# knagrecha/saturn

Measured on AMD Instinct MI355X. Metric: samples_per_s, higher is better.
Workload: dtype bf16; 1 GPU; model=gptj-6b, global_batch=16, seq_len=512, parallelism=dp1, optimizer=fused_sgd

## Files before the change

### saturn_amd/models/gptj.py

```python

from __future__ import annotations


import os
from dataclasses import dataclass

import torch
import torch.nn as nn

from saturn_amd.ops.functional import (
    fused_gelu,
    FusedLayerNorm,
    apply_rope,
    causal_attention,
    fused_add3,
    fused_cross_entropy,
    rope_tables,
    FusedDropout,
    FusedEmbedding,
    gptj_mlp,
    mlp_fused_supported,
)


@dataclass
class GPTJConfig:
    vocab_size: int = 50400
    n_ctx: int = 512
    n_embd: int = 4096
    n_head: int = 16
    n_layer: int = 28
    rotary_dim: int = 64
    embd_pdrop: float = 0.0
    resid_pdrop: float = 0.0


class GPTJAttention(nn.Module):
    def __init__(self, cfg: GPTJConfig):
        super().__init__()
        self.n_head = cfg.n_head
        self.head_dim = cfg.n_embd // cfg.n_head
        self.rotary_dim = cfg.rotary_dim
        E = cfg.n_embd
        self.q_proj = nn.Linear(E, E, bias=False)
        self.k_proj = nn.Linear(E, E, bias=False)
        self.v_proj = nn.Linear(E, E, bias=False)
        self.out_proj = nn.Linear(E, E, bias=False)
        self.n_ctx = cfg.n_ctx
        self._rope_f32 = rope_tables(cfg.n_ctx, cfg.rotary_dim)

    def _rope(self, device):
        if self._rope_f32[0].device != device:
            self._rope_f32 = tuple(t.to(device) for t in self._rope_f32)
        return self._rope_f32

    def forward(self, x):
        B, T, E = x.shape
        H, D = self.n_head, self.head_dim
        q = self.q_proj(x).view(B, T, H, D)
        k = self.k_proj(x).view(B, T, H, D)
        v = self.v_proj(x).view(B, T, H, D)
        cos, sin = self._rope(x.device)
        q = apply_rope(q, cos, sin)
        k = apply_rope(k, cos, sin)
        q = q.transpose(1, 2)
        k = k.transpose(1, 2)
        v = v.transpose(1, 2)
        o = causal_attention(q, k, v)
        o = o.transpose(1, 2).reshape(B, T, -1)
        return self.out_proj(o)


class GPTJMLP(nn.Module):
    def __init__(self, cfg: GPTJConfig):
        super().__init__()
        E = cfg.n_embd
        self.fc_in = nn.Linear(E, 4 * E)
        self.fc_out = nn.Linear(4 * E, E)

    @staticmethod
    def _plain_linear(m) -> bool:
        return type(m) is nn.Linear and not (
            m._forward_hooks
            or m._forward_pre_hooks
            or m._backward_hooks
            or m._backward_pre_hooks
        )

    def _use_fused(self, x) -> bool:
        if os.environ.get("SAMD_MLP_FUSED", "1") == "0":
            return False
        fi, fo = self.fc_in, self.fc_out
        return (
            x.is_cuda
            and self._plain_linear(fi)
            and self._plain_linear(fo)
            and mlp_fused_supported(x, fi.weight, fi.bias, fo.weight, fo.bias)
        )

    def forward(self, x):
        if self._use_fused(x):
            fi, fo = self.fc_in, self.fc_out
            return gptj_mlp(x, fi.weight, fi.bias, fo.weight, fo.bias)
        return self.fc_out(fused_gelu(self.fc_in(x)))


class GPTJBlock(nn.Module):

    def __init__(self, cfg: GPTJConfig):
        super().__init__()
        self.ln_1 = FusedLayerNorm(cfg.n_embd)
        self.attn = GPTJAttention(cfg)
        self.mlp = GPTJMLP(cfg)
        self.drop = FusedDropout(cfg.resid_pdrop)

    def forward(self, x):
        h = self.ln_1(x)
        return fused_add3(x, self.drop(self.attn(h)), self.drop(self.mlp(h)))


class GPTJForCausalLM(nn.Module):
    def __init__(self, cfg: GPTJConfig):
        super().__init__()
        self.cfg = cfg
        self.wte = FusedEmbedding(cfg.vocab_size, cfg.n_embd)
        self.drop = FusedDropout(cfg.embd_pdrop)
        self.h = nn.ModuleList(GPTJBlock(cfg) for _ in range(cfg.n_layer))
        self.ln_f = FusedLayerNorm(cfg.n_embd)
        self.lm_head = nn.Linear(cfg.n_embd, cfg.vocab_size, bias=True)
        self.apply(self._init)

    @staticmethod
    def _init(m):
        if isinstance(m, nn.Linear):
            nn.init.normal_(m.weight, std=0.02)
            if m.bias is not None:
                nn.init.zeros_(m.bias)
        elif isinstance(m, nn.Embedding):
            nn.init.normal_(m.weight, std=0.02)

    def forward(self, input_ids):
        x = self.drop(self.wte(input_ids))
        for block in self.h:
            x = block(x)
        x = self.ln_f(x)
        return self.lm_head(x)


def pretraining_loss(logits, labels):
    return fused_cross_entropy(logits, labels, shift=True)


class _EmbedStage(nn.Module):
    def __init__(self, wte):
        super().__init__()
        self.wte = wte

    def forward(self, input_ids):
        return self.wte(input_ids)


class _HeadStage(nn.Module):
    def __init__(self, ln_f, lm_head):
        super().__init__()
        self.ln_f = ln_f
        self.lm_head = lm_head

    def forward(self, x):
        return self.lm_head(self.ln_f(x))


def as_sequential(model: GPTJForCausalLM) -> nn.Sequential:
    return nn.Sequential(
        _EmbedStage(model.wte), *model.h, _HeadStage(model.ln_f, model.lm_head)
    )


def get_gptj_model(kwargs=None):
    kwargs = kwargs or {}
    cfg = GPTJConfig(
        n_layer=kwargs.get("n_layer", 28),
        n_embd=kwargs.get("n_embd", 4096),
        n_head=kwargs.get("n_head", 16),
        n_ctx=kwargs.get("n_ctx", 512),
        vocab_size=kwargs.get("vocab_size", 50400),
        rotary_dim=kwargs.get("rotary_dim", 64),
        embd_pdrop=kwargs.get("embd_pdrop", 0.0),
        resid_pdrop=kwargs.get("resid_pdrop", 0.0),
    )
    torch.manual_seed(kwargs.get("seed", 0))
    return GPTJForCausalLM(cfg)


class SyntheticTokens(torch.utils.data.Dataset):

    def __init__(self, n: int, seq_len: int, vocab: int, seed: int = 1):
        g = torch.Generator().manual_seed(seed)
        self.data = torch.randint(0, vocab, (n, seq_len), generator=g)

    def __len__(self):
        return len(self.data)

    def __getitem__(self, i):
        return self.data[i]


def _collate(batch):
    x = torch.stack(batch)
    return x, x.clone()


def make_token_dataloader(batch_size=8, seq_len=512, vocab=50400, n_batches=64):
    def get_dataloader():
        return torch.utils.data.DataLoader(
            SyntheticTokens(batch_size * n_batches, seq_len, vocab),
            batch_size=batch_size,
            shuffle=False,
            collate_fn=_collate,
        )

    return get_dataloader
```

### saturn_amd/ops/csrc/bindings.cpp

```cpp

#include <torch/extension.h>
#include <vector>

namespace samd {
void fused_sgd(std::vector<at::Tensor> params, std::vector<at::Tensor> grads,
               std::vector<at::Tensor> moms, std::vector<at::Tensor> masters,
               double lr, double momentum, double weight_decay);
void fused_adam(std::vector<at::Tensor> params, std::vector<at::Tensor> grads,
                std::vector<at::Tensor> ms, std::vector<at::Tensor> vs,
                std::vector<at::Tensor> masters, double lr, double beta1,
                double beta2, double eps, double weight_decay, double bc1,
                double bc2);
std::vector<at::Tensor> norm_fwd(at::Tensor x, at::Tensor w,
                                 c10::optional<at::Tensor> b, double eps,
                                 bool rms);
std::vector<at::Tensor> norm_bwd(at::Tensor dy, at::Tensor x, at::Tensor w,
                                 at::Tensor mean, at::Tensor rstd, bool rms,
                                 bool needs_db);
std::vector<at::Tensor> ce_fwd(at::Tensor logits, at::Tensor targets,
                               int64_t Tr, int64_t ignore_index);
at::Tensor ce_bwd(at::Tensor logits, at::Tensor targets, at::Tensor lse,
                  at::Tensor dloss, int64_t Tr, int64_t ignore_index);
void rope_apply(at::Tensor y, at::Tensor x, at::Tensor cos_t, at::Tensor sin_t,
                int64_t t_len, int64_t t_off, bool half_style, bool backward);
at::Tensor gelu_fwd(at::Tensor x);
at::Tensor gelu_bwd(at::Tensor dy, at::Tensor x);
std::vector<at::Tensor> attn_fwd(at::Tensor q, at::Tensor k, at::Tensor v,
                                 bool causal, int64_t kv_len);
std::vector<at::Tensor> attn_bwd(at::Tensor dout, at::Tensor q, at::Tensor k,
                                 at::Tensor v, at::Tensor o, at::Tensor lse,
                                 bool causal, int64_t kv_len);
std::string attn_dispatch(int64_t T, int64_t D);
at::Tensor add3(at::Tensor a, at::Tensor b, at::Tensor c);
at::Tensor swiglu_fwd(at::Tensor gate, at::Tensor up);
std::vector<at::Tensor> swiglu_bwd(at::Tensor dout, at::Tensor gate,
                                   at::Tensor up);
at::Tensor embed_fwd(at::Tensor weight, at::Tensor idx);
at::Tensor embed_bwd(at::Tensor dout, at::Tensor idx, long vocab);
at::Tensor dropout_fwd(at::Tensor x, double p, long seed);
at::Tensor dropout_bwd(at::Tensor dout, double p, long seed);
std::vector<at::Tensor> moe_route_fwd(at::Tensor logits, int64_t top_k,
                                      at::ScalarType out_dtype);
at::Tensor moe_route_bwd(at::Tensor logits, at::Tensor ids,
                         at::Tensor dweights);
std::vector<at::Tensor> moe_sort(at::Tensor ids, int64_t n_expert);
at::Tensor moe_permute_fwd(at::Tensor x, at::Tensor order, int64_t top_k);
at::Tensor moe_permute_bwd(at::Tensor dxs, at::Tensor pos);
at::Tensor moe_combine_fwd(at::Tensor y, at::Tensor weights, at::Tensor pos);
std::vector<at::Tensor> moe_combine_bwd(at::Tensor dout, at::Tensor y,
                                        at::Tensor weights, at::Tensor pos);
std::vector<at::Tensor> mlp_act_bwd(at::Tensor d_act, at::Tensor pre,
                                    bool want_dT, bool want_aT);
std::vector<at::Tensor> transpose_colsum(at::Tensor x, bool want_sum);
std::vector<at::Tensor> mlp_bwd(at::Tensor g, at::Tensor h, at::Tensor pre,
                                at::Tensor W_in, at::Tensor W_out,
                                bool use_tn_in, bool use_tn_out);
}

PYBIND11_MODULE(TORCH_EXTENSION_NAME, m) {
  m.doc() = "saturn_amd hand-written CDNA4 (gfx950) kernels";
  m.def("fused_sgd", &samd::fused_sgd, "fused multi-tensor SGD");
  m.def("fused_adam", &samd::fused_adam, "fused multi-tensor AdamW");
  m.def("norm_fwd", &samd::norm_fwd, "LayerNorm/RMSNorm forward");
  m.def("norm_bwd", &samd::norm_bwd, "LayerNorm/RMSNorm backward");
  m.def("ce_fwd", &samd::ce_fwd, "fused cross-entropy forward");
  m.def("ce_bwd", &samd::ce_bwd, "fused cross-entropy backward");
  m.def("rope_apply", &samd::rope_apply,
        "fused rotary embedding (out-of-place, offset table rows)");
  m.def("gelu_fwd", &samd::gelu_fwd, "fused tanh-approx GELU forward");
  m.def("gelu_bwd", &samd::gelu_bwd, "fused tanh-approx GELU backward");
  m.def("attn_fwd", &samd::attn_fwd, "fused flash attention forward",
        py::arg("q"), py::arg("k"), py::arg("v"), py::arg("causal"),
        py::arg("kv_len") = -1);
  m.def("attn_dispatch", &samd::attn_dispatch,
        "kernel instantiations attn_fwd/attn_bwd launch for (padded T, D)",
        py::arg("T"), py::arg("D"));
  m.def("attn_bwd", &samd::attn_bwd, "fused flash attention backward",
        py::arg("dout"), py::arg("q"), py::arg("k"), py::arg("v"),
        py::arg("o"), py::arg("lse"), py::arg("causal"),
        py::arg("kv_len") = -1);
  m.def("add3", &samd::add3, "fused 3-way residual add");
  m.def("swiglu_fwd", &samd::swiglu_fwd, "fused silu(gate)*up");
  m.def("swiglu_bwd", &samd::swiglu_bwd, "fused SwiGLU backward");
  m.def("embed_fwd", &samd::embed_fwd, "token embedding gather");
  m.def("embed_bwd", &samd::embed_bwd, "embedding scatter-add backward");
  m.def("dropout_fwd", &samd::dropout_fwd, "counter-based fused dropout");
  m.def("dropout_bwd", &samd::dropout_bwd, "dropout backward (mask recompute)");
  m.def("moe_route_fwd", &samd::moe_route_fwd,
        "MoE softmax + top-k + renormalise (ties to the lower expert)");
  m.def("moe_route_bwd", &samd::moe_route_bwd, "MoE routing backward");
  m.def("moe_sort", &samd::moe_sort,
        "stable counting sort of (token, slot) pairs by expert");
  m.def("moe_permute_fwd", &samd::moe_permute_fwd,
        "gather token rows into expert order");
  m.def("moe_permute_bwd", &samd::moe_permute_bwd,
        "sum each token's k permuted rows");
  m.def("moe_combine_fwd", &samd::moe_combine_fwd,
        "weighted sum of each token's k expert rows");
  m.def("moe_combine_bwd", &samd::moe_combine_bwd,
        "combine backward: dy and fp32 dweights");
  m.def("mlp_act_bwd", &samd::mlp_act_bwd,
        "GELU backward + transposed d_pre / gelu(pre) + fp32 bias grad",
        py::arg("d_act"), py::arg("pre"), py::arg("want_dT") = true,
        py::arg("want_aT") = true);
  m.def("transpose_colsum", &samd::transpose_colsum,
        "bf16 transpose with optional fp32 column sums");
  m.def("mlp_bwd", &samd::mlp_bwd,
        "GPT-J MLP backward with TN-layout weight gradients");
}
```

### saturn_amd/ops/csrc/mlp_bwd.hip

```cpp

#include <torch/extension.h>
#include <ATen/hip/HIPContext.h>

#include "common.h"
#include "gelu_math.h"

namespace samd {

namespace {

constexpr int MB_TILE = 64;
constexpr int MB_ROW_ITERS = 4;
constexpr int MB_BLOCK = 256;

typedef c10::BFloat16 bf16_t;

__device__ __forceinline__ int img_dword(int c, int rp) {
  return c * 32 + (((rp >> 2) ^ (c >> 3)) << 2) + (rp & 3);
}
__device__ __forceinline__ int img_slot(int c, int mv) {
  return c * 8 + (mv ^ (c >> 3));
}

__device__ __forceinline__ float sum8_bf16(const uint4 v) {
  float s = us2f((unsigned short)(v.x & 0xffffu));
  s += us2f((unsigned short)(v.x >> 16));
  s += us2f((unsigned short)(v.y & 0xffffu));
  s += us2f((unsigned short)(v.y >> 16));
  s += us2f((unsigned short)(v.z & 0xffffu));
  s += us2f((unsigned short)(v.z >> 16));
  s += us2f((unsigned short)(v.w & 0xffffu));
  s += us2f((unsigned short)(v.w >> 16));
  return s;
}

__device__ __forceinline__ void store_colsums(float acc0, float acc1,
                                              float4* lds_sum,
                                              float* __restrict__ partial,
                                              long col0, long ncols) {
  const int tid = threadIdx.x;
#pragma unroll
  for (int off = 1; off < 8; off <<= 1) {
    acc0 += __shfl_xor(acc0, off, 64);
    acc1 += __shfl_xor(acc1, off, 64);
  }
  float* s = reinterpret_cast<float*>(lds_sum);
  if ((tid & 7) == 0) {
    s[tid >> 3] = acc0;
    s[(tid >> 3) + 32] = acc1;
  }
  __syncthreads();
  if (tid < MB_TILE / 4 && col0 + tid * 4 < ncols) {
    *reinterpret_cast<float4*>(partial + (long)blockIdx.y * ncols + col0 +
                               tid * 4) = lds_sum[tid];
  }
}

template <bool TN_IN, bool TN_OUT>
__global__ void __launch_bounds__(MB_BLOCK)
mlp_act_bwd_kernel(const bf16_t* __restrict__ d_act,
                   const bf16_t* __restrict__ pre, bf16_t* __restrict__ d_pre,
                   bf16_t* __restrict__ d_preT, bf16_t* __restrict__ act,
                   float* __restrict__ partial, long M, long F) {
  __shared__ uint4 img_d[MB_TILE * 8];
  __shared__ uint4 img_a[TN_OUT ? MB_TILE * 8 : 1];
  __shared__ float4 lds_sum[MB_TILE / 4];

  const int tid = threadIdx.x;
  const int cv = tid & 7;
  const int rp = tid >> 3;
  const int mv = tid & 7;
  const int cr = tid >> 3;
  const long col0 = (long)blockIdx.x * MB_TILE;
  const long col = col0 + cv * 8;
  const bool col_ok = col < F;

  float acc0 = 0.f, acc1 = 0.f;

  for (int it = 0; it < MB_ROW_ITERS; ++it) {
    const long row0 = ((long)blockIdx.y * MB_ROW_ITERS + it) * MB_TILE;
    if (row0 >= M) break;
    const long row = row0 + 2 * rp;
    const bool ok = col_ok && row < M;

    const short8v zero8 = {0, 0, 0, 0, 0, 0, 0, 0};
    short8v xv[2], gv[2];
#pragma unroll
    for (int i = 0; i < 2; ++i) {
      if (ok) {
        const long o = (row + i) * F + col;
        xv[i] = *reinterpret_cast<const short8v*>(pre + o);
        gv[i] = *reinterpret_cast<const short8v*>(d_act + o);
      } else {
        xv[i] = zero8;
        gv[i] = zero8;
      }
    }
    short8v dv[2], av[2];
#pragma unroll
    for (int i = 0; i < 2; ++i) {
#pragma unroll
      for (int e = 0; e < 8; ++e) {
        bf16_t xe, de;
        xe.x = (unsigned short)xv[i][e];
        de.x = (unsigned short)gv[i][e];
        const float xf = toF<bf16_t>(xe);
        dv[i][e] = (short)fromF<bf16_t>(toF<bf16_t>(de) * dgelu_f(xf)).x;
        av[i][e] = (short)fromF<bf16_t>(gelu_f(xf)).x;
      }
    }
    if (ok) {
#pragma unroll
      for (int i = 0; i < 2; ++i) {
        const long o = (row + i) * F + col;
        *reinterpret_cast<short8v*>(d_pre + o) = dv[i];
        if (!TN_OUT) *reinterpret_cast<short8v*>(act + o) = av[i];
      }
    }
    unsigned* d32 = reinterpret_cast<unsigned*>(img_d);
    unsigned* a32 = reinterpret_cast<unsigned*>(img_a);
#pragma unroll
    for (int e = 0; e < 8; ++e) {
      const int w = img_dword(cv * 8 + e, rp);
      d32[w] = ok ? ((unsigned)(unsigned short)dv[0][e] |
                     ((unsigned)(unsigned short)dv[1][e] << 16))
                  : 0u;
      if (TN_OUT)
        a32[w] = ok ? ((unsigned)(unsigned short)av[0][e] |
                       ((unsigned)(unsigned short)av[1][e] << 16))
                    : 0u;
    }
    __syncthreads();

    const long mrow = row0 + mv * 8;
#pragma unroll
    for (int j = 0; j < 2; ++j) {
      const int c = cr + 32 * j;
      const uint4 d = img_d[img_slot(c, mv)];
      const float s = sum8_bf16(d);
      if (j == 0) acc0 += s; else acc1 += s;
      const bool st = (col0 + c < F) && (mrow < M);
      if (TN_IN && st)
        *reinterpret_cast<uint4*>(d_preT + (col0 + c) * M + mrow) = d;
      if (TN_OUT && st)
        *reinterpret_cast<uint4*>(act + (col0 + c) * M + mrow) =
            img_a[img_slot(c, mv)];
    }
    __syncthreads();
  }
  store_colsums(acc0, acc1, lds_sum, partial, col0, F);
}

template <bool SUM, bool STORE>
__global__ void __launch_bounds__(MB_BLOCK)
transpose_colsum_kernel(const bf16_t* __restrict__ x, bf16_t* __restrict__ xT,
                        float* __restrict__ partial, long M, long N) {
  __shared__ uint4 img[MB_TILE * 8];
  __shared__ float4 lds_sum[MB_TILE / 4];

  const int tid = threadIdx.x;
  const int cv = tid & 7;
  const int rp = tid >> 3;
  const int mv = tid & 7;
  const int cr = tid >> 3;
  const long col0 = (long)blockIdx.x * MB_TILE;
  const long col = col0 + cv * 8;
  const bool col_ok = col < N;

  float acc0 = 0.f, acc1 = 0.f;

  for (int it = 0; it < MB_ROW_ITERS; ++it) {
    const long row0 = ((long)blockIdx.y * MB_ROW_ITERS + it) * MB_TILE;
    if (row0 >= M) break;
    const long row = row0 + 2 * rp;
    const bool ok = col_ok && row < M;

    const short8v zero8 = {0, 0, 0, 0, 0, 0, 0, 0};
    short8v xv[2];
#pragma unroll
    for (int i = 0; i < 2; ++i) {
      xv[i] = zero8;
      if (ok) xv[i] = *reinterpret_cast<const short8v*>(x + (row + i) * N + col);
    }
    unsigned* i32 = reinterpret_cast<unsigned*>(img);
#pragma unroll
    for (int e = 0; e < 8; ++e) {
      i32[img_dword(cv * 8 + e, rp)] =
          (unsigned)(unsigned short)xv[0][e] |
          ((unsigned)(unsigned short)xv[1][e] << 16);
    }
    __syncthreads();

    const long mrow = row0 + mv * 8;
#pragma unroll
    for (int j = 0; j < 2; ++j) {
      const int c = cr + 32 * j;
      const uint4 v = img[img_slot(c, mv)];
      if (SUM) {
        const float s = sum8_bf16(v);
        if (j == 0) acc0 += s; else acc1 += s;
      }
      if (STORE && (col0 + c < N) && (mrow < M))
        *reinterpret_cast<uint4*>(xT + (col0 + c) * M + mrow) = v;
    }
    __syncthreads();
  }
  if (SUM) store_colsums(acc0, acc1, lds_sum, partial, col0, N);
}

void check_operand(const at::Tensor& t, const char* name) {
  TORCH_CHECK(t.is_cuda(), name, ": expected a GPU tensor");
  TORCH_CHECK(t.scalar_type() == at::kBFloat16, name, ": expected bf16");
  TORCH_CHECK(t.dim() == 2 && t.is_contiguous(), name,
              ": expected a contiguous 2-D tensor");
  TORCH_CHECK(t.size(0) > 0 && t.size(0) % 8 == 0 && t.size(1) > 0 &&
                  t.size(1) % 8 == 0,
              name, ": both sizes must be positive multiples of 8, got ",
              t.sizes());
  TORCH_CHECK(reinterpret_cast<uintptr_t>(t.data_ptr()) % 16 == 0, name,
              ": data must be 16-byte aligned");
}

dim3 tile_grid(long M, long N) {
  const long gx = (N + MB_TILE - 1) / MB_TILE;
  const long gy = (M + MB_TILE * MB_ROW_ITERS - 1) / (MB_TILE * MB_ROW_ITERS);
  TORCH_CHECK(gy <= 65535, "mlp_bwd: too many rows for one launch");
  return dim3((unsigned)gx, (unsigned)gy);
}

bf16_t* bptr(const at::Tensor& t) {
  return reinterpret_cast<bf16_t*>(t.data_ptr());
}

}

std::vector<at::Tensor> mlp_act_bwd(at::Tensor d_act, at::Tensor pre,
                                    bool want_dT, bool want_aT) {
  check_operand(d_act, "mlp_act_bwd d_act");
  check_operand(pre, "mlp_act_bwd pre");
  TORCH_CHECK(d_act.sizes() == pre.sizes(), "mlp_act_bwd: shape mismatch");
  const long M = pre.size(0), F = pre.size(1);
  auto d_pre = at::empty_like(pre);
  auto d_preT = want_dT ? at::empty({F, M}, pre.options())
                        : at::empty({0}, pre.options());
  auto act = want_aT ? at::empty({F, M}, pre.options()) : at::empty_like(pre);
  const dim3 grid = tile_grid(M, F);
  auto partial =
      at::empty({(long)grid.y, F}, pre.options().dtype(at::kFloat));
  auto stream = at::hip::getCurrentHIPStream();
#define SAMD_LAUNCH_ACT_BWD(TI, TO)                                        \
  hipLaunchKernelGGL((mlp_act_bwd_kernel<TI, TO>), grid, dim3(MB_BLOCK), 0, \
                     stream.stream(), bptr(d_act), bptr(pre), bptr(d_pre),  \
                     want_dT ? bptr(d_preT) : nullptr, bptr(act),           \
                     partial.data_ptr<float>(), M, F)
  if (want_dT && want_aT) SAMD_LAUNCH_ACT_BWD(true, true);
  else if (want_dT) SAMD_LAUNCH_ACT_BWD(true, false);
  else if (want_aT) SAMD_LAUNCH_ACT_BWD(false, true);
  else SAMD_LAUNCH_ACT_BWD(false, false);
#undef SAMD_LAUNCH_ACT_BWD
  SAMD_CHECK_HIP(hipGetLastError());
  return {d_pre, d_preT, act, at::sum(partial, {0})};
}

namespace {

std::vector<at::Tensor> transpose_colsum_impl(const at::Tensor& x,
                                              bool want_sum, bool want_store) {
  check_operand(x, "transpose_colsum x");
  TORCH_CHECK(want_sum || want_store, "transpose_colsum: nothing to do");
  const long M = x.size(0), N = x.size(1);
  auto xT = want_store ? at::empty({N, M}, x.options())
                       : at::empty({0}, x.options());
  const dim3 grid = tile_grid(M, N);
  const auto fopt = x.options().dtype(at::kFloat);
  auto partial = want_sum ? at::empty({(long)grid.y, N}, fopt)
                          : at::empty({0}, fopt);
  auto stream = at::hip::getCurrentHIPStream();
#define SAMD_LAUNCH_TRANSPOSE(SUM, STORE)                                    \
  hipLaunchKernelGGL((transpose_colsum_kernel<SUM, STORE>), grid,            \
                     dim3(MB_BLOCK), 0, stream.stream(), bptr(x),            \
                     want_store ? bptr(xT) : nullptr,                        \
                     want_sum ? partial.data_ptr<float>() : nullptr, M, N)
  if (want_sum && want_store) SAMD_LAUNCH_TRANSPOSE(true, true);
  else if (want_sum) SAMD_LAUNCH_TRANSPOSE(true, false);
  else SAMD_LAUNCH_TRANSPOSE(false, true);
#undef SAMD_LAUNCH_TRANSPOSE
  SAMD_CHECK_HIP(hipGetLastError());
  return {xT, want_sum ? at::sum(partial, {0}) : partial};
}

}

std::vector<at::Tensor> transpose_colsum(at::Tensor x, bool want_sum) {
  return transpose_colsum_impl(x, want_sum, true);
}

std::vector<at::Tensor> mlp_bwd(at::Tensor g, at::Tensor h, at::Tensor pre,
                                at::Tensor W_in, at::Tensor W_out,
                                bool use_tn_in, bool use_tn_out) {
  check_operand(g, "mlp_bwd g");
  check_operand(h, "mlp_bwd h");
  check_operand(pre, "mlp_bwd pre");
  check_operand(W_in, "mlp_bwd W_in");
  check_operand(W_out, "mlp_bwd W_out");
  const long M = g.size(0), E = g.size(1), F = pre.size(1);
  TORCH_CHECK(h.size(0) == M && h.size(1) == E && pre.size(0) == M &&
                  W_in.size(0) == F && W_in.size(1) == E &&
                  W_out.size(0) == E && W_out.size(1) == F,
              "mlp_bwd: inconsistent shapes");

  at::Tensor d_pre, d_preT, act, db_in;
  {
    auto d_act = at::mm(g, W_out);
    auto r = mlp_act_bwd(d_act, pre, use_tn_in, use_tn_out);
    d_pre = r[0];
    d_preT = r[1];
    act = r[2];
    db_in = r[3];
  }
  auto gt = transpose_colsum_impl(g, true, use_tn_out);
  at::Tensor hT;
  if (use_tn_in) hT = transpose_colsum_impl(h, false, true)[0];
  auto dW_out = use_tn_out ? at::linear(gt[0], act) : at::mm(g.t(), act);
  act.reset();
  auto dW_in = use_tn_in ? at::linear(d_preT, hT) : at::mm(d_pre.t(), h);
  d_preT.reset();
  hT.reset();
  auto dh = at::mm(d_pre, W_in);
  return {dh, dW_in, db_in.to(W_in.scalar_type()), dW_out,
          gt[1].to(W_out.scalar_type())};
}

}
```

### saturn_amd/ops/functional.py

```python

from __future__ import annotations

import os
from typing import Tuple

import torch
import torch.nn.functional as F

from saturn_amd.ops import require_ext


class _NormFn(torch.autograd.Function):
    @staticmethod
    def forward(ctx, x, w, b, eps, rms):
        ext = require_ext()
        x = x.contiguous()
        y, mean, rstd = ext.norm_fwd(x, w, b, eps, rms)
        if rms:
            mean = rstd
        ctx.save_for_backward(x, w, mean, rstd)
        ctx.rms = rms
        ctx.has_b = b is not None
        return y

# ... 167 lines not shown
    if cos.shape[0] < off + T:
        raise ValueError(
            "rope table too short for this sequence shard — pass the FULL "
            "table to apply_rope (it slices positions itself)"
        )
    if cos.dtype != torch.float32:
        cos = cos.float()
        sin = sin.float()
    if x.is_cuda:
        return _RopeFn.apply(x, cos.contiguous(), sin.contiguous(), T, off,
                             half_style)
    cos_bt = cos[off : off + T].unsqueeze(0).expand(B, T, half)
    sin_bt = sin[off : off + T].unsqueeze(0).expand(B, T, half)
    return _rope_cpu(x, cos_bt.contiguous(), sin_bt.contiguous(), half_style)


def attention_math(q, k, v, causal: bool = True) -> torch.Tensor:
    scale = 1.0 / (q.shape[-1] ** 0.5)
    s = torch.matmul(q.float(), k.float().transpose(-1, -2)) * scale
    if causal:
        T = q.shape[-2]
        mask = torch.ones(T, T, dtype=torch.bool, device=q.device).tril()
        s = s.masked_fill(~mask, float("-inf"))
    p = torch.softmax(s, dim=-1)
    return torch.matmul(p, v.float()).to(q.dtype)


def _attention_core(q, k, v, causal: bool) -> torch.Tensor:
    if q.is_cuda:
        from saturn_amd.ops import flash

        return flash.flash_attention(q, k, v, causal=causal)
    if k.shape[1] != q.shape[1]:
        rep = q.shape[1] // k.shape[1]
        k = k.repeat_interleave(rep, dim=1)
        v = v.repeat_interleave(rep, dim=1)
    return attention_math(q, k, v, causal=causal)


def _attention(q, k, v, causal: bool) -> torch.Tensor:
    from saturn_amd.parallel.sequence import sp_attention, sp_world

    if sp_world() > 1:
        return sp_attention(q, k, v, lambda a, b, c: _attention_core(a, b, c, causal))
    return _attention_core(q, k, v, causal)


def causal_attention(q, k, v) -> torch.Tensor:
    return _attention(q, k, v, causal=True)


def full_attention(q, k, v) -> torch.Tensor:
    return _attention(q, k, v, causal=False)


class _Add3Fn(torch.autograd.Function):
    @staticmethod
    def forward(ctx, a, b, c):
        ext = require_ext()
        return ext.add3(a.contiguous(), b.contiguous(), c.contiguous())

    @staticmethod
    def backward(ctx, g):
        return g, g, g


def fused_add3(a, b, c):
    if a.is_cuda:
        return _Add3Fn.apply(a, b, c)
    return a + b + c


class _GeluFn(torch.autograd.Function):
    @staticmethod
    def forward(ctx, x):
        ext = require_ext()
        x = x.contiguous()
        ctx.save_for_backward(x)
        return ext.gelu_fwd(x)

    @staticmethod
    def backward(ctx, dy):
        ext = require_ext()
        (x,) = ctx.saved_tensors
        return ext.gelu_bwd(dy.contiguous(), x)


def fused_gelu(x: torch.Tensor) -> torch.Tensor:
    if x.is_cuda and x.dtype in (torch.bfloat16, torch.float16):
        return _GeluFn.apply(x)
    return torch.nn.functional.gelu(x, approximate="tanh")


_MLP_TN_DEFAULT = {"in": True, "out": True}


def _mlp_tn(site: str) -> bool:
    v = os.environ.get("SAMD_MLP_TN_" + site.upper())
    return _MLP_TN_DEFAULT[site] if v is None else v != "0"


def mlp_fused_supported(x, w_in, b_in, w_out, b_out) -> bool:
    if not (x.is_cuda and x.dtype == torch.bfloat16 and x.dim() >= 2):
        return False
    if b_in is None or b_out is None:
        return False
    if any(t.dtype != torch.bfloat16 or not t.is_cuda
           for t in (w_in, b_in, w_out, b_out)):
        return False
    E = x.shape[-1]
    M = x.numel() // E if E else 0
    F_ = w_in.shape[0]
    return (
        M > 0
        and w_in.shape == (F_, E)
        and w_out.shape == (E, F_)
        and M % 8 == 0
        and E % 8 == 0
        and F_ % 8 == 0
    )


class _GPTJMlpFn(torch.autograd.Function):

    @staticmethod
    def forward(ctx, h, w_in, b_in, w_out, b_out):
        ext = require_ext()
        pre = F.linear(h, w_in, b_in).contiguous()
        out = F.linear(ext.gelu_fwd(pre), w_out, b_out)
        ctx.save_for_backward(h, pre, w_in, w_out)
        return out

    @staticmethod
    def backward(ctx, g):
        ext = require_ext()
        h, pre, w_in, w_out = ctx.saved_tensors
        E = h.shape[-1]
        dh, dw_in, db_in, dw_out, db_out = ext.mlp_bwd(
            g.contiguous().view(-1, E),
            h.contiguous().view(-1, E),
            pre.view(-1, pre.shape[-1]),
            w_in.contiguous(),
            w_out.contiguous(),
            _mlp_tn("in"),
            _mlp_tn("out"),
        )
        return dh.view(h.shape), dw_in, db_in, dw_out, db_out


def gptj_mlp(h, w_in, b_in, w_out, b_out):
    return _GPTJMlpFn.apply(h, w_in, b_in, w_out, b_out)


class _SwigluFn(torch.autograd.Function):
    @staticmethod
    def forward(ctx, gate, up):
        ext = require_ext()
        gate = gate.contiguous()
        up = up.contiguous()
        ctx.save_for_backward(gate, up)
        return ext.swiglu_fwd(gate, up)

    @staticmethod
    def backward(ctx, dout):
        ext = require_ext()
        gate, up = ctx.saved_tensors
        dgate, dup = ext.swiglu_bwd(dout.contiguous(), gate, up)
        return dgate, dup


def fused_swiglu(gate, up):
    if gate.is_cuda:
        return _SwigluFn.apply(gate, up)
    return torch.nn.functional.silu(gate) * up


class _EmbedFn(torch.autograd.Function):
    @staticmethod
    def forward(ctx, weight, idx):
        ext = require_ext()
        ctx.save_for_backward(idx)
        ctx.vocab = weight.shape[0]
        return ext.embed_fwd(weight, idx)

    @staticmethod
    def backward(ctx, dout):
        ext = require_ext()
        (idx,) = ctx.saved_tensors
        return ext.embed_bwd(dout, idx, ctx.vocab), None


def fused_embedding(weight, idx):
    if weight.is_cuda:
        return _EmbedFn.apply(weight, idx)
    return F.embedding(idx, weight)


class FusedEmbedding(torch.nn.Embedding):

    def forward(self, idx):
        if (
            self.weight.is_cuda
            and self.padding_idx is None
            and self.max_norm is None
            and not self.sparse
            and self.weight.dtype
            in (torch.bfloat16, torch.float16, torch.float32)
        ):
            return _EmbedFn.apply(self.weight, idx)
        return super().forward(idx)


class _DropoutFn(torch.autograd.Function):
    @staticmethod
    def forward(ctx, x, p, seed):
        ext = require_ext()
        ctx.p = p
        ctx.seed = seed
        return ext.dropout_fwd(x, p, seed)

    @staticmethod
    def backward(ctx, dout):
        ext = require_ext()
        return ext.dropout_bwd(dout.contiguous(), ctx.p, ctx.seed), None, None


def fused_dropout(x, p: float, training: bool = True):
    if p == 0.0 or not training:
        return x
    if x.is_cuda and x.dtype in (torch.bfloat16, torch.float16):
        seed = int(torch.randint(0, 2**62, (1,)).item())
        return _DropoutFn.apply(x.contiguous(), p, seed)
    return F.dropout(x, p, training)


class FusedDropout(torch.nn.Module):
    def __init__(self, p: float = 0.0):
        super().__init__()
        self.p = p

    def forward(self, x):
        return fused_dropout(x, self.p, self.training)

    def extra_repr(self):
        return f"p={self.p}"
```

### setup.py

```python

import os

from setuptools import setup

os.environ.setdefault("PYTORCH_ROCM_ARCH", "gfx950")

from torch.utils.cpp_extension import BuildExtension, CUDAExtension

CSRC = os.path.join("saturn_amd", "ops", "csrc")

ext = CUDAExtension(
    name="saturn_amd._C",
    sources=[
        os.path.join(CSRC, "bindings.cpp"),
        os.path.join(CSRC, "fused_optim.hip"),
        os.path.join(CSRC, "layernorm.hip"),
        os.path.join(CSRC, "cross_entropy.hip"),
        os.path.join(CSRC, "rope.hip"),
        os.path.join(CSRC, "gelu.hip"),
        os.path.join(CSRC, "attention.hip"),
        os.path.join(CSRC, "add3.hip"),
        os.path.join(CSRC, "swiglu.hip"),
        os.path.join(CSRC, "embedding.hip"),
        os.path.join(CSRC, "dropout.hip"),
        os.path.join(CSRC, "moe.hip"),
        os.path.join(CSRC, "mlp_bwd.hip"),
    ],
    extra_compile_args={
        "cxx": ["-O3", "-std=c++17"],
        "nvcc": ["-O3", "-std=c++17", "--offload-arch=gfx950"],
    },
)

comm_ext = CUDAExtension(
    name="saturn_amd._comm",
    sources=[os.path.join("saturn_amd", "comm", "csrc", "rccl_comm.cpp")],
    libraries=["rccl"],
    extra_compile_args={
        "cxx": ["-O3", "-std=c++17"],
        "nvcc": ["-O3", "-std=c++17", "--offload-arch=gfx950"],
    },
)

setup(
    name="saturn_amd",
    version="0.1.0",
    packages=[
        "saturn_amd",
        "saturn_amd.core",
        "saturn_amd.library",
        "saturn_amd.solver",
        "saturn_amd.engine",
        "saturn_amd.trial_runner",
        "saturn_amd.executors",
        "saturn_amd.parallel",
        "saturn_amd.ops",
        "saturn_amd.comm",
        "saturn_amd.models",
        "saturn_amd.utils",
    ],
    ext_modules=[ext, comm_ext],
    cmdclass={"build_ext": BuildExtension},
)
```

Measured before the change: 62.36 samples/s.

## Fuse GPT-J attention and MLP branch backward with shared transposes

```diff
diff --git a/saturn_amd/models/gptj.py b/saturn_amd/models/gptj.py
--- a/saturn_amd/models/gptj.py
+++ b/saturn_amd/models/gptj.py
@@ -20,6 +20,8 @@
     FusedEmbedding,
     gptj_mlp,
     mlp_fused_supported,
+    gptj_branches,
+    gptj_branches_supported,
 )
 
 
@@ -114,8 +116,58 @@
         self.mlp = GPTJMLP(cfg)
         self.drop = FusedDropout(cfg.resid_pdrop)
 
+    @staticmethod
+    def _hooked(m) -> bool:
+        return bool(
+            m._forward_hooks
+            or m._forward_pre_hooks
+            or m._backward_hooks
+            or m._backward_pre_hooks
+        )
+
+    def _use_fused(self, h) -> bool:
+        if (os.environ.get("SAMD_MLP_FUSED", "1") == "0"
+                or os.environ.get("SAMD_BLOCK_FUSED", "1") == "0"):
+            return False
+        attn, mlp = self.attn, self.mlp
+        if type(attn) is not GPTJAttention or type(mlp) is not GPTJMLP:
+            return False
+        if not (h.is_cuda and h.dtype == torch.bfloat16 and h.dim() == 3):
+            return False
+        if self.drop.p != 0.0:
+            return False
+        from saturn_amd.parallel.sequence import sp_world
+
+        if sp_world() != 1:
+            return False
+        if any(self._hooked(m) for b in (attn, mlp, self.drop) for m in b.modules()):
+            return False
+        projs = (attn.q_proj, attn.k_proj, attn.v_proj, attn.out_proj)
+        fi, fo = mlp.fc_in, mlp.fc_out
+        if not all(GPTJMLP._plain_linear(m) for m in (*projs, fi, fo)):
+            return False
+        E = h.shape[-1]
+        if any(m.bias is not None or m.weight.shape != (E, E)
+               or m.weight.dtype != torch.bfloat16 or not m.weight.is_cuda
+               for m in projs):
+            return False
+        return mlp_fused_supported(
+            h, fi.weight, fi.bias, fo.weight, fo.bias
+        ) and gptj_branches_supported(
+            h, attn.n_head, attn.rotary_dim, attn._rope_f32[0].shape[0]
+        )
+
     def forward(self, x):
         h = self.ln_1(x)
+        if self._use_fused(h):
+            attn, mlp = self.attn, self.mlp
+            cos, sin = attn._rope(h.device)
+            a, m = gptj_branches(
+                h, attn.q_proj.weight, attn.k_proj.weight, attn.v_proj.weight,
+                attn.out_proj.weight, mlp.fc_in.weight, mlp.fc_in.bias,
+                mlp.fc_out.weight, mlp.fc_out.bias, cos, sin, attn.n_head,
+            )
+            return fused_add3(x, a, m)
         return fused_add3(x, self.drop(self.attn(h)), self.drop(self.mlp(h)))
 
 
diff --git a/saturn_amd/ops/csrc/bindings.cpp b/saturn_amd/ops/csrc/bindings.cpp
--- a/saturn_amd/ops/csrc/bindings.cpp
+++ b/saturn_amd/ops/csrc/bindings.cpp
@@ -55,6 +55,16 @@
 std::vector<at::Tensor> mlp_bwd(at::Tensor g, at::Tensor h, at::Tensor pre,
                                 at::Tensor W_in, at::Tensor W_out,
                                 bool use_tn_in, bool use_tn_out);
+void transpose_into(at::Tensor x, at::Tensor dst);
+at::Tensor rope_bwd_t(at::Tensor dy, at::Tensor cos_t, at::Tensor sin_t,
+                      int64_t t_len, int64_t t_off, int64_t dim,
+                      at::Tensor dxT);
+std::vector<at::Tensor> gptj_branches_bwd(
+    at::Tensor g_a, at::Tensor g_m, at::Tensor h, at::Tensor pre, at::Tensor q,
+    at::Tensor k, at::Tensor v, at::Tensor o, at::Tensor lse, at::Tensor Wq,
+    at::Tensor Wk, at::Tensor Wv, at::Tensor Wo, at::Tensor W_in,
+    at::Tensor W_out, at::Tensor cos_t, at::Tensor sin_t, int64_t t_off,
+    bool tn_in, bool tn_out, bool tn_qkv, bool tn_o, bool dh_accum);
 }
 
 PYBIND11_MODULE(TORCH_EXTENSION_NAME, m) {
@@ -107,4 +117,13 @@
         "bf16 transpose with optional fp32 column sums");
   m.def("mlp_bwd", &samd::mlp_bwd,
         "GPT-J MLP backward with TN-layout weight gradients");
+  m.def("transpose_into", &samd::transpose_into,
+        "bf16 transpose stored into a caller-given [N, M] view",
+        py::arg("x"), py::arg("dst"));
+  m.def("rope_bwd_t", &samd::rope_bwd_t,
+        "interleaved RoPE backward that also stores dx^T into a [E, M] view",
+        py::arg("dy"), py::arg("cos"), py::arg("sin"), py::arg("t_len"),
+        py::arg("t_off"), py::arg("dim"), py::arg("dxT"));
+  m.def("gptj_branches_bwd", &samd::gptj_branches_bwd,
+        "GPT-J attention + MLP branch backward with shared transposes");
 }
diff --git a/saturn_amd/ops/csrc/gptj_block_bwd.hip b/saturn_amd/ops/csrc/gptj_block_bwd.hip
--- /dev/null
+++ b/saturn_amd/ops/csrc/gptj_block_bwd.hip
@@ -0,0 +1,269 @@
+
+#include <torch/extension.h>
+#include <ATen/hip/HIPContext.h>
+
+#include "common.h"
+#include "tile_image.h"
+
+namespace samd {
+
+std::vector<at::Tensor> attn_bwd(at::Tensor dout, at::Tensor q, at::Tensor k,
+                                 at::Tensor v, at::Tensor o, at::Tensor lse,
+                                 bool causal, int64_t kv_len);
+std::vector<at::Tensor> mlp_act_bwd(at::Tensor d_act, at::Tensor pre,
+                                    bool want_dT, bool want_aT);
+void rope_apply(at::Tensor y, at::Tensor x, at::Tensor cos_t, at::Tensor sin_t,
+                int64_t t_len, int64_t t_off, bool half_style, bool backward);
+
+namespace {
+
+__global__ void __launch_bounds__(MB_BLOCK)
+rope_bwd_t_kernel(const bf16_t* __restrict__ dy, bf16_t* __restrict__ dx,
+                  bf16_t* __restrict__ dxT, const float* __restrict__ cos_t,
+                  const float* __restrict__ sin_t, long M, long E, int t_len,
+                  long t_off, int dim, int half, float sign) {
+  __shared__ uint4 img[MB_TILE * 8];
+
+  const int tid = threadIdx.x;
+  const int cv = tid & 7;
+  const int rp = tid >> 3;
+  const int mv = tid & 7;
+  const int cr = tid >> 3;
+  const long col0 = (long)blockIdx.x * MB_TILE;
+  const long col = col0 + cv * 8;
+  const bool col_ok = col < E;
+  const int j0 = (int)(col % dim);
+  const bool rotary = j0 < 2 * half;
+
+  for (int it = 0; it < MB_ROW_ITERS; ++it) {
+    const long row0 = ((long)blockIdx.y * MB_ROW_ITERS + it) * MB_TILE;
+    if (row0 >= M) break;
+    const long row = row0 + 2 * rp;
+    const bool ok = col_ok && row < M;
+
+    const short8v zero8 = {0, 0, 0, 0, 0, 0, 0, 0};
+    short8v ov[2];
+#pragma unroll
+    for (int i = 0; i < 2; ++i) {
+      ov[i] = zero8;
+      if (!ok) continue;
+      const short8v xv =
+          *reinterpret_cast<const short8v*>(dy + (row + i) * E + col);
+      if (rotary) {
+        const long trow = (t_off + ((row + i) % t_len)) * (long)half;
+#pragma unroll
+        for (int e = 0; e < 4; ++e) {
+          const int p = j0 / 2 + e;
+          const float c = cos_t[trow + p];
+          const float s = sin_t[trow + p] * sign;
+          bf16_t e0, e1;
+          e0.x = (unsigned short)xv[2 * e];
+          e1.x = (unsigned short)xv[2 * e + 1];
+          const float x0 = toF<bf16_t>(e0);
+          const float x1 = toF<bf16_t>(e1);
+          ov[i][2 * e] = (short)fromF<bf16_t>(x0 * c - x1 * s).x;
+          ov[i][2 * e + 1] = (short)fromF<bf16_t>(x1 * c + x0 * s).x;
+        }
+      } else {
+        ov[i] = xv;
+      }
+      *reinterpret_cast<short8v*>(dx + (row + i) * E + col) = ov[i];
+    }
+    unsigned* i32 = reinterpret_cast<unsigned*>(img);
+#pragma unroll
+    for (int e = 0; e < 8; ++e) {
+      i32[img_dword(cv * 8 + e, rp)] =
+          (unsigned)(unsigned short)ov[0][e] |
+          ((unsigned)(unsigned short)ov[1][e] << 16);
+    }
+    __syncthreads();
+
+    const long mrow = row0 + mv * 8;
+#pragma unroll
+    for (int j = 0; j < 2; ++j) {
+      const int c = cr + 32 * j;
+      if ((col0 + c < E) && (mrow < M))
+        *reinterpret_cast<uint4*>(dxT + (col0 + c) * M + mrow) =
+            img[img_slot(c, mv)];
+    }
+    __syncthreads();
+  }
+}
+
+void check_f32_table(const at::Tensor& t, const char* name) {
+  TORCH_CHECK(t.is_cuda() && t.scalar_type() == at::kFloat && t.dim() == 2 &&
+                  t.is_contiguous(),
+              name, ": expected a contiguous fp32 [T, half] GPU tensor");
+}
+
+}
+
+at::Tensor rope_bwd_t(at::Tensor dy, at::Tensor cos_t, at::Tensor sin_t,
+                      int64_t t_len, int64_t t_off, int64_t dim,
+                      at::Tensor dxT) {
+  TORCH_CHECK(dy.is_cuda() && dy.scalar_type() == at::kBFloat16 &&
+                  dy.is_contiguous() && dy.numel() > 0,
+              "rope_bwd_t dy: expected a contiguous bf16 GPU tensor");
+  check_f32_table(cos_t, "rope_bwd_t cos");
+  check_f32_table(sin_t, "rope_bwd_t sin");
+  const long half = cos_t.size(1);
+  TORCH_CHECK(sin_t.sizes() == cos_t.sizes(), "rope_bwd_t: table mismatch");
+  TORCH_CHECK(dim > 0 && dim % 8 == 0, "rope_bwd_t: head dim ", dim,
+              " must be a positive multiple of 8");
+  TORCH_CHECK((2 * half) % 8 == 0 && 2 * half <= dim,
+              "rope_bwd_t: rotary dim ", 2 * half,
+              " must be a multiple of 8 within the head dim");
+  TORCH_CHECK(dy.numel() % dim == 0 && dy.size(-1) == dim,
+              "rope_bwd_t: last dim of dy must be the head dim");
+  TORCH_CHECK(dy.dim() >= 2, "rope_bwd_t dy: expected [..., heads, dim]");
+  const long E = dy.size(-2) * dim;
+  const long M = dy.numel() / E;
+  TORCH_CHECK(M % 8 == 0, "rope_bwd_t: token count ", M,
+              " must be a multiple of 8");
+  TORCH_CHECK(t_len > 0 && M % t_len == 0,
+              "rope_bwd_t: token count not a multiple of T");
+  TORCH_CHECK(t_off >= 0 && cos_t.size(0) >= t_off + t_len,
+              "rope_bwd_t: table too short for offset+T");
+  TORCH_CHECK(reinterpret_cast<uintptr_t>(dy.data_ptr()) % 16 == 0,
+              "rope_bwd_t dy: data must be 16-byte aligned");
+  check_operand(dxT, "rope_bwd_t dxT");
+  TORCH_CHECK(dxT.size(0) == E && dxT.size(1) == M &&
+                  dxT.device() == dy.device(),
+              "rope_bwd_t: dxT must be [", E, ", ", M, "], got ", dxT.sizes());
+
+  auto dx = at::empty_like(dy);
+  const dim3 grid = tile_grid(M, E);
+  auto stream = at::hip::getCurrentHIPStream();
+  hipLaunchKernelGGL(rope_bwd_t_kernel, grid, dim3(MB_BLOCK), 0,
+                     stream.stream(), bptr(dy), bptr(dx), bptr(dxT),
+                     cos_t.data_ptr<float>(), sin_t.data_ptr<float>(), M, E,
+                     (int)t_len, (long)t_off, (int)dim, (int)half, -1.f);
+  SAMD_CHECK_HIP(hipGetLastError());
+  return dx;
+}
+
+std::vector<at::Tensor> gptj_branches_bwd(
+    at::Tensor g_a, at::Tensor g_m, at::Tensor h, at::Tensor pre, at::Tensor q,
+    at::Tensor k, at::Tensor v, at::Tensor o, at::Tensor lse, at::Tensor Wq,
+    at::Tensor Wk, at::Tensor Wv, at::Tensor Wo, at::Tensor W_in,
+    at::Tensor W_out, at::Tensor cos_t, at::Tensor sin_t, int64_t t_off,
+    bool tn_in, bool tn_out, bool tn_qkv, bool tn_o, bool dh_accum) {
+  check_operand(g_a, "gptj_branches_bwd g_a");
+  check_operand(g_m, "gptj_branches_bwd g_m");
+  check_operand(h, "gptj_branches_bwd h");
+  check_operand(pre, "gptj_branches_bwd pre");
+  check_operand(W_in, "gptj_branches_bwd W_in");
+  check_operand(W_out, "gptj_branches_bwd W_out");
+  const long M = h.size(0), E = h.size(1), F = pre.size(1);
+  TORCH_CHECK(q.dim() == 4 && o.dim() == 4, "gptj_branches_bwd: q, o 4-D");
+  const long B = q.size(0), H = q.size(1), T = q.size(2), D = q.size(3);
+  TORCH_CHECK(B * T == M && H * D == E && k.sizes() == q.sizes() &&
+                  v.sizes() == q.sizes() && o.sizes() == q.sizes(),
+              "gptj_branches_bwd: attention shapes do not match h");
+  TORCH_CHECK(g_a.sizes() == h.sizes() && g_m.sizes() == h.sizes() &&
+                  pre.size(0) == M && W_in.size(0) == F && W_in.size(1) == E &&
+                  W_out.size(0) == E && W_out.size(1) == F,
+              "gptj_branches_bwd: inconsistent shapes");
+  for (const at::Tensor* w : {&Wq, &Wk, &Wv, &Wo}) {
+    check_operand(*w, "gptj_branches_bwd projection weight");
+    TORCH_CHECK(w->size(0) == E && w->size(1) == E,
+                "gptj_branches_bwd: projection weights must be [E, E]");
+  }
+  auto o_phys = o.permute({0, 2, 1, 3});
+  TORCH_CHECK(o_phys.is_contiguous(),
+              "gptj_branches_bwd: o must be physically [B,T,H,D]");
+  auto o2 = o_phys.view({M, E});
+  const bool shared = g_a.data_ptr() == g_m.data_ptr();
+
+  auto gt = transpose_colsum_impl(g_m, true, tn_out || (shared && tn_o));
+  at::Tensor gaT;
+  if (tn_o) gaT = shared ? gt[0] : transpose_colsum_impl(g_a, false, true)[0];
+  at::Tensor hT;
+  if (tn_in || tn_qkv) hT = transpose_colsum_impl(h, false, true)[0];
+
+  at::Tensor dh, dW_in, db_in, dW_out;
+  {
+    at::Tensor d_pre, d_preT, act;
+    {
+      auto d_act = at::mm(g_m, W_out);
+      auto r = mlp_act_bwd(d_act, pre, tn_in, tn_out);
+      d_pre = r[0];
+      d_preT = r[1];
+      act = r[2];
+      db_in = r[3];
+    }
+    dW_out = tn_out ? at::linear(gt[0], act) : at::mm(g_m.t(), act);
+    act.reset();
+    if (!tn_o) gt[0].reset();
+    dW_in = tn_in ? at::linear(d_preT, hT) : at::mm(d_pre.t(), h);
+    d_preT.reset();
+    if (!tn_qkv) hT.reset();
+    dh = at::mm(d_pre, W_in);
+  }
+
+  auto d_o = at::mm(g_a, Wo);
+  at::Tensor dWo;
+  if (tn_o) {
+    auto oT = transpose_colsum_impl(o2, false, true)[0];
+    dWo = at::linear(gaT, oT);
+    gaT.reset();
+    gt[0].reset();
+  } else {
+    dWo = at::mm(g_a.t(), o2);
+  }
+
+  at::Tensor dq_r, dk_r, dv;
+  {
+    auto r = attn_bwd(d_o.view({B, T, H, D}).permute({0, 2, 1, 3}), q, k, v, o,
+                      lse, true, T);
+    dq_r = r[0].permute({0, 2, 1, 3});
+    dk_r = r[1].permute({0, 2, 1, 3});
+    dv = r[2].permute({0, 2, 1, 3});
+    TORCH_CHECK(dq_r.is_contiguous() && dk_r.is_contiguous() &&
+                    dv.is_contiguous(),
+                "gptj_branches_bwd: attn_bwd layout changed");
+  }
+  d_o.reset();
+  auto dv2 = dv.view({M, E});
+
+  at::Tensor dq, dk, dWq, dWk, dWv;
+  if (tn_qkv) {
+    auto dqkvT = at::empty({3 * E, M}, h.options());
+    dq = rope_bwd_t(dq_r, cos_t, sin_t, T, t_off, D, dqkvT.narrow(0, 0, E));
+    dq_r.reset();
+    dk = rope_bwd_t(dk_r, cos_t, sin_t, T, t_off, D, dqkvT.narrow(0, E, E));
+    dk_r.reset();
+    transpose_colsum_impl(dv2, false, true, dqkvT.narrow(0, 2 * E, E));
+    auto dW = at::linear(dqkvT, hT);
+    dqkvT.reset();
+    hT.reset();
+    dWq = dW.narrow(0, 0, E);
+    dWk = dW.narrow(0, E, E);
+    dWv = dW.narrow(0, 2 * E, E);
+  } else {
+    dq = at::empty_like(dq_r);
+    rope_apply(dq, dq_r, cos_t, sin_t, T, t_off, false, true);
+    dq_r.reset();
+    dk = at::empty_like(dk_r);
+    rope_apply(dk, dk_r, cos_t, sin_t, T, t_off, false, true);
+    dk_r.reset();
+    dWq = at::mm(dq.view({M, E}).t(), h);
+    dWk = at::mm(dk.view({M, E}).t(), h);
+    dWv = at::mm(dv2.t(), h);
+  }
+
+  auto dq2 = dq.view({M, E}), dk2 = dk.view({M, E});
+  if (dh_accum) {
+    dh.addmm_(dv2, Wv);
+    dh.addmm_(dk2, Wk);
+    dh.addmm_(dq2, Wq);
+  } else {
+    dh.add_(at::mm(dv2, Wv));
+    dh.add_(at::mm(dk2, Wk));
+    dh.add_(at::mm(dq2, Wq));
+  }
+  return {dh, dWq, dWk, dWv, dWo, dW_in, db_in.to(W_in.scalar_type()),
+          dW_out, gt[1].to(W_out.scalar_type())};
+}
+
+}
diff --git a/saturn_amd/ops/csrc/mlp_bwd.hip b/saturn_amd/ops/csrc/mlp_bwd.hip
--- a/saturn_amd/ops/csrc/mlp_bwd.hip
+++ b/saturn_amd/ops/csrc/mlp_bwd.hip
@@ -4,57 +4,11 @@
 
 #include "common.h"
 #include "gelu_math.h"
+#include "tile_image.h"
 
 namespace samd {
 
 namespace {
-
-constexpr int MB_TILE = 64;
-constexpr int MB_ROW_ITERS = 4;
-constexpr int MB_BLOCK = 256;
-
-typedef c10::BFloat16 bf16_t;
-
-__device__ __forceinline__ int img_dword(int c, int rp) {
-  return c * 32 + (((rp >> 2) ^ (c >> 3)) << 2) + (rp & 3);
-}
-__device__ __forceinline__ int img_slot(int c, int mv) {
-  return c * 8 + (mv ^ (c >> 3));
-}
-
-__device__ __forceinline__ float sum8_bf16(const uint4 v) {
-  float s = us2f((unsigned short)(v.x & 0xffffu));
-  s += us2f((unsigned short)(v.x >> 16));
-  s += us2f((unsigned short)(v.y & 0xffffu));
-  s += us2f((unsigned short)(v.y >> 16));
-  s += us2f((unsigned short)(v.z & 0xffffu));
-  s += us2f((unsigned short)(v.z >> 16));
-  s += us2f((unsigned short)(v.w & 0xffffu));
-  s += us2f((unsigned short)(v.w >> 16));
-  return s;
-}
-
-__device__ __forceinline__ void store_colsums(float acc0, float acc1,
-                                              float4* lds_sum,
-                                              float* __restrict__ partial,
-                                              long col0, long ncols) {
-  const int tid = threadIdx.x;
-#pragma unroll
-  for (int off = 1; off < 8; off <<= 1) {
-    acc0 += __shfl_xor(acc0, off, 64);
-    acc1 += __shfl_xor(acc1, off, 64);
-  }
-  float* s = reinterpret_cast<float*>(lds_sum);
-  if ((tid & 7) == 0) {
-    s[tid >> 3] = acc0;
-    s[(tid >> 3) + 32] = acc1;
-  }
-  __syncthreads();
-  if (tid < MB_TILE / 4 && col0 + tid * 4 < ncols) {
-    *reinterpret_cast<float4*>(partial + (long)blockIdx.y * ncols + col0 +
-                               tid * 4) = lds_sum[tid];
-  }
-}
 
 template <bool TN_IN, bool TN_OUT>
 __global__ void __launch_bounds__(MB_BLOCK)
@@ -206,30 +160,6 @@
     __syncthreads();
   }
   if (SUM) store_colsums(acc0, acc1, lds_sum, partial, col0, N);
-}
-
-void check_operand(const at::Tensor& t, const char* name) {
-  TORCH_CHECK(t.is_cuda(), name, ": expected a GPU tensor");
-  TORCH_CHECK(t.scalar_type() == at::kBFloat16, name, ": expected bf16");
-  TORCH_CHECK(t.dim() == 2 && t.is_contiguous(), name,
-              ": expected a contiguous 2-D tensor");
-  TORCH_CHECK(t.size(0) > 0 && t.size(0) % 8 == 0 && t.size(1) > 0 &&
-                  t.size(1) % 8 == 0,
-              name, ": both sizes must be positive multiples of 8, got ",
-              t.sizes());
-  TORCH_CHECK(reinterpret_cast<uintptr_t>(t.data_ptr()) % 16 == 0, name,
-              ": data must be 16-byte aligned");
-}
-
-dim3 tile_grid(long M, long N) {
-  const long gx = (N + MB_TILE - 1) / MB_TILE;
-  const long gy = (M + MB_TILE * MB_ROW_ITERS - 1) / (MB_TILE * MB_ROW_ITERS);
-  TORCH_CHECK(gy <= 65535, "mlp_bwd: too many rows for one launch");
-  return dim3((unsigned)gx, (unsigned)gy);
-}
-
-bf16_t* bptr(const at::Tensor& t) {
-  return reinterpret_cast<bf16_t*>(t.data_ptr());
 }
 
 }
@@ -262,15 +192,24 @@
   return {d_pre, d_preT, act, at::sum(partial, {0})};
 }
 
-namespace {
-
-std::vector<at::Tensor> transpose_colsum_impl(const at::Tensor& x,
-                                              bool want_sum, bool want_store) {
+std::vector<at::Tensor> transpose_colsum_impl(
+    const at::Tensor& x, bool want_sum, bool want_store,
+    const c10::optional<at::Tensor>& dst) {
   check_operand(x, "transpose_colsum x");
   TORCH_CHECK(want_sum || want_store, "transpose_colsum: nothing to do");
   const long M = x.size(0), N = x.size(1);
-  auto xT = want_store ? at::empty({N, M}, x.options())
-                       : at::empty({0}, x.options());
+  at::Tensor xT;
+  if (want_store && dst.has_value()) {
+    xT = *dst;
+    check_operand(xT, "transpose_colsum dst");
+    TORCH_CHECK(xT.size(0) == N && xT.size(1) == M &&
+                    xT.device() == x.device(),
+                "transpose_colsum: dst must be [", N, ", ", M, "], got ",
+                xT.sizes());
+  } else {
+    xT = want_store ? at::empty({N, M}, x.options())
+                    : at::empty({0}, x.options());
+  }
   const dim3 grid = tile_grid(M, N);
   const auto fopt = x.options().dtype(at::kFloat);
   auto partial = want_sum ? at::empty({(long)grid.y, N}, fopt)
@@ -289,10 +228,12 @@
   return {xT, want_sum ? at::sum(partial, {0}) : partial};
 }
 
-}
-
 std::vector<at::Tensor> transpose_colsum(at::Tensor x, bool want_sum) {
   return transpose_colsum_impl(x, want_sum, true);
+}
+
+void transpose_into(at::Tensor x, at::Tensor dst) {
+  transpose_colsum_impl(x, false, true, dst);
 }
 
 std::vector<at::Tensor> mlp_bwd(at::Tensor g, at::Tensor h, at::Tensor pre,
diff --git a/saturn_amd/ops/csrc/tile_image.h b/saturn_amd/ops/csrc/tile_image.h
--- /dev/null
+++ b/saturn_amd/ops/csrc/tile_image.h
@@ -0,0 +1,86 @@
+#pragma once
+
+#include <torch/extension.h>
+
+#include <vector>
+
+#include "common.h"
+
+namespace samd {
+
+constexpr int MB_TILE = 64;
+constexpr int MB_ROW_ITERS = 4;
+constexpr int MB_BLOCK = 256;
+
+typedef c10::BFloat16 bf16_t;
+
+__device__ __forceinline__ int img_dword(int c, int rp) {
+  return c * 32 + (((rp >> 2) ^ (c >> 3)) << 2) + (rp & 3);
+}
+__device__ __forceinline__ int img_slot(int c, int mv) {
+  return c * 8 + (mv ^ (c >> 3));
+}
+
+__device__ __forceinline__ float sum8_bf16(const uint4 v) {
+  float s = us2f((unsigned short)(v.x & 0xffffu));
+  s += us2f((unsigned short)(v.x >> 16));
+  s += us2f((unsigned short)(v.y & 0xffffu));
+  s += us2f((unsigned short)(v.y >> 16));
+  s += us2f((unsigned short)(v.z & 0xffffu));
+  s += us2f((unsigned short)(v.z >> 16));
+  s += us2f((unsigned short)(v.w & 0xffffu));
+  s += us2f((unsigned short)(v.w >> 16));
+  return s;
+}
+
+__device__ __forceinline__ void store_colsums(float acc0, float acc1,
+                                              float4* lds_sum,
+                                              float* __restrict__ partial,
+                                              long col0, long ncols) {
+  const int tid = threadIdx.x;
+#pragma unroll
+  for (int off = 1; off < 8; off <<= 1) {
+    acc0 += __shfl_xor(acc0, off, 64);
+    acc1 += __shfl_xor(acc1, off, 64);
+  }
+  float* s = reinterpret_cast<float*>(lds_sum);
+  if ((tid & 7) == 0) {
+    s[tid >> 3] = acc0;
+    s[(tid >> 3) + 32] = acc1;
+  }
+  __syncthreads();
+  if (tid < MB_TILE / 4 && col0 + tid * 4 < ncols) {
+    *reinterpret_cast<float4*>(partial + (long)blockIdx.y * ncols + col0 +
+                               tid * 4) = lds_sum[tid];
+  }
+}
+
+inline void check_operand(const at::Tensor& t, const char* name) {
+  TORCH_CHECK(t.is_cuda(), name, ": expected a GPU tensor");
+  TORCH_CHECK(t.scalar_type() == at::kBFloat16, name, ": expected bf16");
+  TORCH_CHECK(t.dim() == 2 && t.is_contiguous(), name,
+              ": expected a contiguous 2-D tensor");
+  TORCH_CHECK(t.size(0) > 0 && t.size(0) % 8 == 0 && t.size(1) > 0 &&
+                  t.size(1) % 8 == 0,
+              name, ": both sizes must be positive multiples of 8, got ",
+              t.sizes());
+  TORCH_CHECK(reinterpret_cast<uintptr_t>(t.data_ptr()) % 16 == 0, name,
+              ": data must be 16-byte aligned");
+}
+
+inline dim3 tile_grid(long M, long N) {
+  const long gx = (N + MB_TILE - 1) / MB_TILE;
+  const long gy = (M + MB_TILE * MB_ROW_ITERS - 1) / (MB_TILE * MB_ROW_ITERS);
+  TORCH_CHECK(gy <= 65535, "mlp_bwd: too many rows for one launch");
+  return dim3((unsigned)gx, (unsigned)gy);
+}
+
+inline bf16_t* bptr(const at::Tensor& t) {
+  return reinterpret_cast<bf16_t*>(t.data_ptr());
+}
+
+std::vector<at::Tensor> transpose_colsum_impl(
+    const at::Tensor& x, bool want_sum, bool want_store,
+    const c10::optional<at::Tensor>& dst = c10::nullopt);
+
+}
diff --git a/saturn_amd/ops/functional.py b/saturn_amd/ops/functional.py
--- a/saturn_amd/ops/functional.py
+++ b/saturn_amd/ops/functional.py
@@ -343,6 +343,109 @@
     return _GPTJMlpFn.apply(h, w_in, b_in, w_out, b_out)
 
 
+_BLOCK_SITE_DEFAULT = {
+    "SAMD_ATTN_TN_QKV": True,
+    "SAMD_ATTN_TN_OUT": True,
+    "SAMD_DH_ACCUM": False,
+}
+
+
+def _block_site(name: str) -> bool:
+    v = os.environ.get(name)
+    return _BLOCK_SITE_DEFAULT[name] if v is None else v != "0"
+
+
+def _same_tensor(a, b) -> bool:
+    return (
+        a.data_ptr() == b.data_ptr()
+        and a.shape == b.shape
+        and a.stride() == b.stride()
+    )
+
+
+class _GPTJBranchesFn(torch.autograd.Function):
+
+    @staticmethod
+    def forward(ctx, h, wq, wk, wv, wo, w_in, b_in, w_out, b_out, cos, sin,
+                n_head, t_off):
+        ext = require_ext()
+        B, T, E = h.shape
+        D = E // n_head
+        q = F.linear(h, wq).view(B, T, n_head, D)
+        k = F.linear(h, wk).view(B, T, n_head, D)
+        v = F.linear(h, wv).view(B, T, n_head, D)
+        qr = torch.empty_like(q)
+        ext.rope_apply(qr, q, cos, sin, T, t_off, False, False)
+        kr = torch.empty_like(k)
+        ext.rope_apply(kr, k, cos, sin, T, t_off, False, False)
+        del q, k
+        qr, kr, v = qr.transpose(1, 2), kr.transpose(1, 2), v.transpose(1, 2)
+        o, lse = ext.attn_fwd(qr, kr, v, True, T)
+        attn_out = F.linear(o.transpose(1, 2).reshape(B, T, E), wo)
+        pre = F.linear(h, w_in, b_in).contiguous()
+        mlp_out = F.linear(ext.gelu_fwd(pre), w_out, b_out)
+        ctx.save_for_backward(h, pre, qr, kr, v, o, lse, wq, wk, wv, wo,
+                              w_in, w_out, cos, sin)
+        ctx.t_off = t_off
+        return attn_out, mlp_out
+
+    @staticmethod
+    def backward(ctx, g_a, g_m):
+        ext = require_ext()
+        (h, pre, qr, kr, v, o, lse, wq, wk, wv, wo, w_in, w_out, cos,
+         sin) = ctx.saved_tensors
+        E = h.shape[-1]
+        if g_a is None:
+            g_a = torch.zeros_like(h)
+        if g_m is None:
+            g_m = torch.zeros_like(h)
+        if _same_tensor(g_a, g_m):
+            g_a = g_m = g_m.contiguous().view(-1, E)
+        else:
+            g_a = g_a.contiguous().view(-1, E)
+            g_m = g_m.contiguous().view(-1, E)
+        dh, dwq, dwk, dwv, dwo, dw_in, db_in, dw_out, db_out = (
+            ext.gptj_branches_bwd(
+                g_a, g_m,
+                h.contiguous().view(-1, E),
+                pre.view(-1, pre.shape[-1]),
+                qr, kr, v, o, lse,
+                wq.contiguous(), wk.contiguous(), wv.contiguous(),
+                wo.contiguous(), w_in.contiguous(), w_out.contiguous(),
+                cos, sin, ctx.t_off,
+                _mlp_tn("in"), _mlp_tn("out"),
+                _block_site("SAMD_ATTN_TN_QKV"),
+                _block_site("SAMD_ATTN_TN_OUT"),
+                _block_site("SAMD_DH_ACCUM"),
+            )
+        )
+        return (dh.view(h.shape), dwq, dwk, dwv, dwo, dw_in, db_in, dw_out,
+                db_out, None, None, None, None)
+
+
+def gptj_branches_supported(h, n_head, rotary_dim, table_len) -> bool:
+    if h.dim() != 3 or n_head <= 0:
+        return False
+    B, T, E = h.shape
+    if E % n_head:
+        return False
+    D = E // n_head
+    return (
+        T % 64 == 0
+        and T <= table_len
+        and D in (64, 128, 256)
+        and rotary_dim > 0
+        and rotary_dim % 8 == 0
+        and rotary_dim <= D
+    )
+
+
+def gptj_branches(h, wq, wk, wv, wo, w_in, b_in, w_out, b_out, cos, sin,
+                  n_head):
+    return _GPTJBranchesFn.apply(h, wq, wk, wv, wo, w_in, b_in, w_out, b_out,
+                                 cos.contiguous(), sin.contiguous(), n_head, 0)
+
+
 class _SwigluFn(torch.autograd.Function):
     @staticmethod
     def forward(ctx, gate, up):
diff --git a/setup.py b/setup.py
--- a/setup.py
+++ b/setup.py
@@ -25,6 +25,7 @@
         os.path.join(CSRC, "dropout.hip"),
         os.path.join(CSRC, "moe.hip"),
         os.path.join(CSRC, "mlp_bwd.hip"),
+        os.path.join(CSRC, "gptj_block_bwd.hip"),
     ],
     extra_compile_args={
         "cxx": ["-O3", "-std=c++17"],
```

New measurement: 64.23 samples/s, median of 6. +3.0%, better.
